# noveens/reviews4rec

Measured on AMD Instinct MI355X. Metric: train ratings/sec, higher is better.
Workload: dtype f32

## Files before the change

### include/r4r.h

```cpp
#ifndef R4R_H
#define R4R_H

#include <stddef.h>
#include <stdint.h>

#ifdef __cplusplus
extern "C" {
#endif

#define R4R_OK 0
#define R4R_ERR_ARG (-1)
#define R4R_ERR_LAUNCH (-2)
#define R4R_ERR_WORKSPACE (-3)

int r4r_version(void);
const char *r4r_last_error(void);

size_t r4r_textcnn_ws_bytes(int64_t N, int T, int E, int F, int64_t V);
int r4r_textcnn_fwd(const float *table, int64_t V, const int64_t *idx,
                    const float *conv_w, const float *conv_b,
                    float *pooled, int32_t *argmax,
                    void *ws, size_t ws_bytes,
                    int64_t N, int T, int E, int F, void *stream);

// ... 13 lines not shown
                      void *ws, size_t ws_bytes,
                      int64_t N, int T, int E, int F, void *stream);

int r4r_linear_fwd(const float *x, const float *w, const float *b, float *y,
                   int64_t N, int n_in, int n_out, int relu, void *stream);
size_t r4r_linear_bwd_ws_bytes(int64_t N, int n_in, int n_out);
int r4r_linear_bwd(const float *x, const float *w, const float *y, const float *g_y,
                   float *g_x, float *g_w, float *g_b, void *ws, size_t ws_bytes,
                   int64_t N, int n_in, int n_out, int relu, void *stream);

int r4r_dropout_fwd(const float *x, float *y, float *mult, int64_t n, float p,
                    uint64_t seed, uint64_t offset, uint64_t *offset_dev, void *stream);
int r4r_counter_add(uint64_t *counter, uint64_t delta, void *stream);
int r4r_mul(const float *a, const float *b, float *out, int64_t n, void *stream);
int r4r_add(const float *a, const float *b, float *out, int64_t n, void *stream);

int r4r_fm_fwd(const float *x, const float *V, const float *lin_w, const float *lin_b,
               float *out, int64_t N, int n, int k, void *stream);
int r4r_fm_bwd(const float *x, const float *V, const float *lin_w, const float *g_out,
               float *g_x, float *g_V, float *g_lin_w, float *g_lin_b,
               int64_t N, int n, int k, void *stream);

int r4r_embed_gather(const float *table, const int64_t *idx, float *out,
                     int64_t R, int D, int64_t n, void *stream);
int r4r_embed_scatter_add(const float *g_out, const int64_t *idx, float *g_table,
                          int64_t R, int D, int64_t n, void *stream);
int r4r_embed_scatter_add_ordered(const float *g_out, const int64_t *idx, float *g_table,
                                  int64_t R, int D, int64_t n, void *stream);

int r4r_rowdot_fwd(const float *a, const float *c, float *out, int64_t N, int D, void *stream);
int r4r_rowdot_bwd(const float *a, const float *c, const float *g_out, float *g_a, float *g_c,
                   int64_t N, int D, void *stream);
int r4r_bias_head_fwd(const float *r, const float *user_bias, const float *item_bias,
                      const float *global_bias, const int64_t *uid, const int64_t *iid,
                      float *out, int64_t N, void *stream);
int r4r_bias_head_bwd(const float *g_out, const int64_t *uid, const int64_t *iid,
                      float *g_user_bias, float *g_item_bias, float *g_global,
                      int64_t RU, int64_t RI, int64_t N, void *stream);

size_t r4r_narre_attn_ws_bytes(int64_t N, int R, int L);
int r4r_narre_attn_fwd(const float *x, const float *other, const float *W0, const float *b0,
                       const float *w3, const float *b3, const float *mult,
                       float *out, float *h_save, float *a_save,
                       int64_t N, int R, int L, void *stream);
int r4r_narre_attn_bwd(const float *x, const float *other, const float *W0, const float *w3,
                       const float *mult, const float *h_save, const float *a_save,
                       const float *g_out,
                       float *g_x, float *g_other, float *g_W0, float *g_b0, float *g_w3, float *g_b3,
                       void *ws, size_t ws_bytes,
                       int64_t N, int R, int L, void *stream);

int r4r_mse_fwd_bwd(const float *out, const float *y, float *se, float *g_out,
                    int64_t N, float denom, void *stream);

int r4r_sqdist_mean_fwd(const float *a, const float *b, float *out, int64_t N, int L, void *stream);
int r4r_sqdist_mean_bwd(const float *a, const float *b, const float *g_out, float *g_a, float *g_b,
                        int64_t N, int L, void *stream);

int r4r_adam_chunk_elems(void);
int r4r_adam_multi(int ntensor, const uint64_t *p, const uint64_t *g, const uint64_t *m, const uint64_t *v,
                   const int64_t *numel, float lr, double beta1, double beta2, float eps,
                   float weight_decay, int64_t step, const int64_t *step_dev, void *stream);
int r4r_adam_gathered(float *p, const float *gathered, int world, float *g_sum, float *m, float *v,
                      int64_t numel, float lr, double beta1, double beta2, float eps,
                      float weight_decay, int64_t step, void *stream);
int r4r_adam_gathered_guarded(float *p, const float *gathered, int world, float *g_sum, float *m, float *v,
                              int64_t numel, float lr, double beta1, double beta2, float eps,
                              float weight_decay, int64_t step, const uint32_t *abort_word, void *stream);

int r4r_peer_segment_create(int64_t bytes, void **ptr, uint8_t *handle);
int r4r_peer_segment_open(const uint8_t *handle, void **ptr);
int r4r_peer_segment_close(void *ptr);
int r4r_peer_segment_destroy(void *ptr);
int r4r_peer_push(const float *src, int64_t numel, const uint64_t *peer_dst, const uint64_t *peer_flags,
                  uint32_t *arrive, int rank, int world, uint32_t epoch, const uint32_t *wait_flags,
                  uint32_t *timed_out, double timeout_s, void *stream);
int r4r_peer_wait(const uint32_t *flags, int world, uint32_t epoch, uint32_t *timed_out, double timeout_s, void *stream);


#define R4R_CONV_AUTO 0
#define R4R_CONV_DIRECT 1
#define R4R_CONV_PROJECT 2
int r4r_deepconn_nparam(void);
int r4r_deepconn_layout(int E, int L, int64_t *offsets, int64_t *sizes, int64_t *total);
size_t r4r_deepconn_ws_bytes(int64_t B, int T, int E, int L, int64_t V);
size_t r4r_deepconn_ws_mult_offset(int64_t B, int T, int E, int L, int64_t V);
size_t r4r_deepconn_ws_count_offset(int64_t B, int T, int E, int L, int64_t V, int tower, int buffer);
int r4r_deepconn_step(const float *table, int64_t V, const int64_t *user_idx, const int64_t *item_idx,
                      const float *y, float *flat_p, float *flat_g,
                      float *pred, float *se, float *sse_accum,
                      void *ws, size_t ws_bytes,
                      int64_t B, int T, int E, int L,
                      float dropout_p, int training, uint64_t seed, uint64_t offset,
                      float inv_denom, int conv_algo, int token_buffer, int tokens_ready,
                      const int64_t *next_user_idx, const int64_t *next_item_idx,
                      float *flat_m, float *flat_v, float lr, double beta1, double beta2, float eps,
                      float weight_decay, int64_t adam_step, void *stream);
int r4r_deepconn_tokens(const int64_t *user_idx, const int64_t *item_idx, void *ws, size_t ws_bytes,
                        int64_t B, int T, int E, int L, int64_t V, int conv_algo, int token_buffer,
                        int discard, void *stream);

#define R4R_TIMING_TEXTCNN_FWD 0
#define R4R_TIMING_TEXTCNN_WGRAD 1
#define R4R_TIMING_ADAM 2
#define R4R_TIMING_PROJ_GEMM 3
#define R4R_TIMING_PROJ_GATHER 4
#define R4R_TIMING_SLOTS 8
int r4r_timing_enable(int slot_mask);
int r4r_timing_read(int slot, double *total_ms, int64_t *count, int reset);

size_t r4r_mf_ws_bytes(int64_t B, int D, int64_t n_users, int64_t n_items);
size_t r4r_mf_ws_persist_bytes(int64_t B, int D, int64_t n_users, int64_t n_items);
size_t r4r_mf_ws_mult_offset(int64_t B, int D, int64_t n_users, int64_t n_items);
size_t r4r_mf_ws_grad_offset(int64_t B, int D, int64_t n_users, int64_t n_items, int which);
int r4r_mf_step(const int64_t *uid, const int64_t *iid, const float *y,
                const uint64_t *p, const uint64_t *m, const uint64_t *v,
                int64_t n_users, int64_t n_items, int D,
                float *pred, float *se, float *sse_accum, void *ws, size_t ws_bytes, int64_t B,
                float dropout_p, int training, uint64_t seed, uint64_t offset, float inv_denom,
                int sweep_period, int64_t sweep_base, int sweep_all,
                float lr, double beta1, double beta2, float eps, float weight_decay, int64_t adam_step,
                void *stream);

int r4r_mf_rows_flush(const uint64_t *p, const uint64_t *m, const uint64_t *v,
                      int64_t n_users, int64_t n_items, int D, void *ws, size_t ws_bytes, int64_t B,
                      int sweep_period, int64_t sweep_base,
                      float lr, double beta1, double beta2, float eps, float weight_decay, int64_t adam_step,
                      void *stream);
size_t r4r_mf_ws_flag_offset(int64_t B, int D, int64_t n_users, int64_t n_items);

int r4r_sse_accumulate(const float *se, int64_t n, float *accum, void *stream);

size_t r4r_mf_dp_block_bytes(int64_t B_pad, int D);
int r4r_mf_grad(const int64_t *uid, const int64_t *iid, const float *y, const uint64_t *p,
                const uint64_t *m, const uint64_t *v,
                int64_t n_users, int64_t n_items, int D, float *pred, float *se, void *block, float *mult,
                int64_t B, int64_t B_pad, float dropout_p, int training, uint64_t seed, uint64_t offset,
                float inv_denom, void *ws, int sweep_period, int64_t sweep_base,
                float lr, double beta1, double beta2, float eps, float weight_decay, int64_t adam_step,
                void *stream);
int r4r_mf_apply(const void *blocks, int world, int64_t B_pad, const uint64_t *p, const uint64_t *m,
                 const uint64_t *v, int64_t n_users, int64_t n_items, int D, void *ws, size_t ws_bytes,
                 int sweep_period, int64_t sweep_base, int sweep_all,
                 const float *se, int64_t se_n, float *sse_accum,
                 float lr, double beta1, double beta2, float eps, float weight_decay, int64_t adam_step,
                 void *stream);
int r4r_mf_grad_push(const int64_t *uid, const int64_t *iid, const float *y, const uint64_t *p,
                     const uint64_t *m, const uint64_t *v,
                     int64_t n_users, int64_t n_items, int D, float *pred, float *se, float *mult,
                     int64_t B, int64_t B_pad, float dropout_p, int training, uint64_t seed, uint64_t offset,
                     float inv_denom, void *ws, int sweep_period, int64_t sweep_base,
                     float lr, double beta1, double beta2, float eps, float weight_decay, int64_t adam_step,
                     const uint64_t *peer_dst, const uint64_t *peer_flags, uint32_t *arrive, int rank, int world,
                     uint32_t epoch, void *stream);
int r4r_mf_apply_peer(const void *blocks, int world, int64_t B_pad, const uint64_t *p, const uint64_t *m,
                      const uint64_t *v, int64_t n_users, int64_t n_items, int D, void *ws, size_t ws_bytes,
                      int sweep_period, int64_t sweep_base, int sweep_all,
                      const float *se, int64_t se_n, float *sse_accum,
                      float lr, double beta1, double beta2, float eps, float weight_decay, int64_t adam_step,
                      const uint32_t *wait_flags, uint32_t epoch, uint32_t *timed_out, double timeout_s,
                      void *stream);

size_t r4r_dp_block_bytes(int nfields, const int *widths, int64_t B_pad);
int r4r_dp_pack(int nfields, const uint64_t *src, const int *widths, const int *pad_ones, int64_t n,
                int64_t B_pad, void *block, void *stream);
int r4r_dp_unpack(int nfields, const uint64_t *dst, const int *widths, const void *blocks, int world,
// ... 268 lines not shown
```

### reviews4rec_amd/csrc/engine.hip

```cpp
#include <stdlib.h>

#include "trace_device.h"
#include "textcnn.h"
#include "wgrad_device.h"
#include "tokens_device.h"
#include "adam_device.h"

namespace r4r {

constexpr int F_CONV = 100;
constexpr int FM_K = 8;
constexpr int MAX_L = 128;

enum { P_UCW = 0, P_UCB, P_UFW, P_UFB, P_ICW, P_ICB, P_IFW, P_IFB, P_FMV, P_FMLW, P_FMLB, P_GB, P_COUNT };

struct Layout {
    int64_t off[P_COUNT], size[P_COUNT], total;
};

static Layout make_layout(int E, int L) {
    Layout lay;
    const int64_t sz[P_COUNT] = {(int64_t)F_CONV * 3 * E, F_CONV, (int64_t)L * F_CONV, L,
                                 (int64_t)F_CONV * 3 * E, F_CONV, (int64_t)L * F_CONV, L,
                                 (int64_t)2 * L * FM_K, 2 * L, 1, 1};
    int64_t o = 0;
    for (int i = 0; i < P_COUNT; ++i) {
        lay.off[i] = o;
        lay.size[i] = sz[i];
        o += (sz[i] + 31) & ~(int64_t)31;
    }
    lay.total = o;
    return lay;
}

struct HeadArgs {
    const float *pmax[2]; const int *parg[2];
    const float *fc_w[2]; const float *fc_b[2];
    const float *V, *lin_w, *lin_b, *gbias;
    const float *y;
    float *pooled[2]; int *argmax[2];
    float *g_pooled[2];
    float *mult;
    float *x, *s, *g, *gz;
    float *pred, *se;
    int64_t B;
    int L, tiles, training, want_grad;
    float p_drop, inv_denom;
    uint64_t seed, offset;
};


constexpr int HEAD_MAX_TILES = 8;

#define SEL2(arr, s) ((s) ? (arr)[1] : (arr)[0])
HEAD_TRACE_DEFINE(r4r_debug_dc_head_trace)
template <int ML>
__global__ __launch_bounds__(256) void deepconn_head_wg_kernel(HeadArgs a) {
    HEAD_STAMP(0)
    constexpr int N2 = 2 * ML, PARTS = 256 / N2;
    __shared__ float sw[2][ML][F_CONV + 1];
    __shared__ float sfb[N2], slw[N2], sz[N2];
    __shared__ float sV[N2][FM_K];
    __shared__ float sp[2][F_CONV + 4];
    __shared__ float red[N2][PARTS + 1];
    const int tid = threadIdx.x, lane = tid & 63, w = tid >> 6;
    const int64_t b = blockIdx.x;
    const int L = a.L, n = 2 * L;
    const float lin_b0 = a.lin_b[0], gbias0 = a.gbias[0], yb = a.y ? a.y[b] : 0.f;

    constexpr int FQ = F_CONV / 4;
    typedef float hq4 __attribute__((ext_vector_type(4)));
    constexpr int WREGS = (2 * ML * FQ + 255) / 256;
    hq4 wreg[WREGS];
    const int wtot = 2 * L * FQ;
#pragma unroll
    for (int k = 0; k < WREGS; ++k) {
        const int i = min(tid + 256 * k, wtot - 1);
        const int t = i >= L * FQ;
        wreg[k] = *reinterpret_cast<const hq4 *>(SEL2(a.fc_w, t) + 4 * (i - t * L * FQ));
    }
    const int tn = min(tid, n - 1);
    const float fbreg = SEL2(a.fc_b, tn >= L)[tn - (tn >= L ? L : 0)];
    const float lwreg = a.lin_w[tn];
    constexpr int VREGS = (N2 * FM_K + 255) / 256;
    float vreg[VREGS];
#pragma unroll
    for (int k = 0; k < VREGS; ++k) vreg[k] = a.V[min(tid + 256 * k, n * FM_K - 1)];

    {
        const int t = w >> 1, f = lane + 64 * (w & 1), fc = min(f, F_CONV - 1);
        float best = -INFINITY;
        int bp = -1;
        if (a.tiles <= HEAD_MAX_TILES) {
            float v[HEAD_MAX_TILES];
            int pp[HEAD_MAX_TILES];
#pragma unroll
            for (int k = 0; k < HEAD_MAX_TILES; ++k) {
                const size_t o = ((size_t)b * a.tiles + min(k, a.tiles - 1)) * NP + fc;
                v[k] = SEL2(a.pmax, t)[o];
                pp[k] = SEL2(a.parg, t)[o];
            }
#pragma unroll
            for (int k = 0; k < HEAD_MAX_TILES; ++k)
                if (v[k] > best) { best = v[k]; bp = pp[k]; }
        } else {
            for (int k0 = 0; k0 < a.tiles; k0 += HEAD_MAX_TILES) {
                float v[HEAD_MAX_TILES];
                int pp[HEAD_MAX_TILES];
#pragma unroll
                for (int k = 0; k < HEAD_MAX_TILES; ++k) {
                    const bool in = k0 + k < a.tiles;
                    const size_t o = ((size_t)b * a.tiles + (in ? k0 + k : 0)) * NP + fc;
                    v[k] = in ? SEL2(a.pmax, t)[o] : -INFINITY;
                    pp[k] = SEL2(a.parg, t)[o];
                }
#pragma unroll
                for (int k = 0; k < HEAD_MAX_TILES; ++k)
                    if (v[k] > best) { best = v[k]; bp = pp[k]; }
            }
        }
        if (!(best > 0.f)) { best = 0.f; bp = -1; }
        if (f < F_CONV) {
            sp[t][f] = best;
            SEL2(a.pooled, t)[b * F_CONV + f] = best;
            SEL2(a.argmax, t)[b * F_CONV + f] = bp;
        }
    }
    HEAD_STAMP(1)
#pragma unroll
    for (int k = 0; k < WREGS; ++k) {
        const int i = tid + 256 * k;
        if (i < wtot) {
            const int t = i >= L * FQ, r = i - t * L * FQ, l = r / FQ, f0 = 4 * (r - l * FQ);
#pragma unroll
            for (int c = 0; c < 4; ++c) sw[t][l][f0 + c] = wreg[k][c];
        }
    }
    if (tid < n) { sfb[tid] = fbreg; slw[tid] = lwreg; }
#pragma unroll
    for (int k = 0; k < VREGS; ++k) {
// ... 19 lines not shown
        float xi[NI], mult[NI], lw[NI], gacc[NI];
#pragma unroll
        for (int u = 0; u < NI; ++u) {
            const int i = lane + 64 * u;
            xi[u] = 0.f; mult[u] = 1.f; gacc[u] = 0.f;
            lw[u] = (i < n) ? slw[i] : 0.f;
            if (i < n) {
                float acc = 0.f;
#pragma unroll
                for (int q = 0; q < PARTS; ++q) acc += red[i][q];
                xi[u] = acc + sfb[i];
            }
            if (a.training && a.p_drop > 0.f && i < n) {
                const uint32_t r = philox_first_word(a.offset + (uint64_t)(b * n + i), a.seed);
                const float uu = (float)(r >> 8) * (1.0f / 16777216.0f);
                mult[u] = (uu >= a.p_drop) ? 1.f / (1.f - a.p_drop) : 0.f;
            }
            xi[u] *= mult[u];
        }
        float inter = 0.f;
        float sk_keep[FM_K];
#pragma unroll
        for (int k = 0; k < FM_K; ++k) {
            float pv = 0.f, pv2 = 0.f, vv[NI];
#pragma unroll
            for (int u = 0; u < NI; ++u) {
                const int i = lane + 64 * u;
                vv[u] = (i < n) ? sV[i][k] : 0.f;
                pv += xi[u] * vv[u];
                pv2 += xi[u] * xi[u] * vv[u] * vv[u];
            }
            const float sk = wave_sum(pv);
            const float s2 = wave_sum(pv2);
            inter += sk * sk - s2;
#pragma unroll
            for (int u = 0; u < NI; ++u) gacc[u] += sk * vv[u] - xi[u] * vv[u] * vv[u];
            sk_keep[k] = sk;
        }
        float pl = 0.f;
#pragma unroll
        for (int u = 0; u < NI; ++u) pl += xi[u] * lw[u];
        const float lin = wave_sum(pl);
        const float pred = (0.5f * inter + lin + lin_b0) + gbias0;
        if (lane == 0) a.pred[b] = pred;
        if (has_y) {
            const float d = pred - yb;
            if (lane == 0) a.se[b] = d * d;
            if (want) {
                const float g = 2.f * d * a.inv_denom;
#pragma unroll
                for (int u = 0; u < NI; ++u) {
                    const int i = lane + 64 * u;
                    const float gx = g * (gacc[u] + lw[u]);
                    const float gz = gx * mult[u];
                    if (i < n) {
                        sz[i] = gz;
                        a.x[b * n + i] = xi[u];
                        a.gz[b * n + i] = gz;
                        a.mult[b * n + i] = mult[u];
                    }
                }
                if (lane < FM_K) {
                    float sv = 0.f;
#pragma unroll
                    for (int k = 0; k < FM_K; ++k) if (lane == k) sv = sk_keep[k];
                    a.s[b * FM_K + lane] = sv;
                }
                if (lane == 0) a.g[b] = g;
            }
        }
    }
    if (!want) return;
    __syncthreads();
    HEAD_STAMP(3)
    if (tid < 2 * F_CONV) {
        const int t = tid >= F_CONV, f = tid - t * F_CONV;
        float acc = 0.f;
        for (int l = 0; l < L; ++l) acc = fmaf(sz[t * L + l], sw[t][l][f], acc);
        SEL2(a.g_pooled, t)[b * F_CONV + f] = acc;
    }
    HEAD_STAMP(4)
}

struct HeadGradArgs {
    const float *pooled[2];
    const float *x, *s, *g, *gz;
    const float *V;
    const float *se;
    float *g_fc_w[2], *g_fc_b[2], *g_V, *g_lin_w, *g_lin_b, *g_gb;
    float *sse_accum;
    int64_t B;
    int L;
};

constexpr int HG_ROWS = 16, HG_COLS = 16;
__device__ __forceinline__ void head_grad_block(const HeadGradArgs &a, int blk) {
    __shared__ float red[HG_ROWS][HG_COLS];
    const int ox = threadIdx.x & (HG_COLS - 1), rg = threadIdx.x / HG_COLS;
    const int L = a.L, n = 2 * L;
    const int n_fcw = L * F_CONV;
    const int seg[9] = {n_fcw, L, n_fcw, L, n * FM_K, n, 1, 1, 1};
    int o = blk * HG_COLS + ox;
    int which = -1, local = 0, acc_o = o;
#pragma unroll
    for (int k = 0; k < 9; ++k) {
        if (which < 0) {
            if (acc_o < seg[k]) { which = k; local = acc_o; }
            else acc_o -= seg[k];
        }
    }
    float s = 0.f;
    if (which >= 0) {
        const bool is_w = which == 0 || which == 2, is_b = which == 1 || which == 3, is_v = which == 4, is_lw = which == 5;
        const int t = which >> 1;
        const int wl = local / F_CONV, wf = local - wl * F_CONV;
        const int vi = local / FM_K, vk = local - vi * FM_K;
        const float *pa = (is_w || is_b) ? a.gz : (which == 8 ? a.se : a.g);
        const int64_t sa = (is_w || is_b) ? n : 1;
        const int64_t oa = is_w ? t * L + wl : (is_b ? t * L + local : 0);
        const bool useb = is_w || is_v, usec = is_v || is_lw;
        const float *pb = is_w ? a.pooled[t & 1] : (is_v ? a.s : a.g);
        const int64_t sb = is_w ? F_CONV : (is_v ? FM_K : 1), ob = is_w ? wf : (is_v ? vk : 0);
        const float *pc = usec ? a.x : a.g;
        const int64_t sc = usec ? n : 1, oc = is_v ? vi : (is_lw ? local : 0);
        const float cv = is_v ? a.V[local] : 0.f;
        constexpr int HB = 8;
        for (int64_t b0 = rg; b0 < a.B; b0 += (int64_t)HG_ROWS * HB) {
            float va[HB], vb[HB], vc[HB];
#pragma unroll
            for (int k = 0; k < HB; ++k) {
                const int64_t b = min(b0 + (int64_t)k * HG_ROWS, a.B - 1);
                va[k] = pa[b * sa + oa];
                vb[k] = pb[b * sb + ob];
                vc[k] = pc[b * sc + oc];
            }
#pragma unroll
            for (int k = 0; k < HB; ++k) {
                const float B_ = useb ? vb[k] : 1.f, C_ = usec ? vc[k] : 1.f;
                const float term = va[k] * (B_ * C_ - C_ * C_ * cv);
                if (b0 + (int64_t)k * HG_ROWS < a.B) s += term;
            }
        }
    }
    red[rg][ox] = s;
    __syncthreads();
    if (rg == 0 && which >= 0) {
        float t = 0.f;
#pragma unroll
        for (int r = 0; r < HG_ROWS; ++r) t += red[r][ox];
        switch (which) {
            case 0: a.g_fc_w[0][local] = t; break;
            case 1: a.g_fc_b[0][local] = t; break;
            case 2: a.g_fc_w[1][local] = t; break;
            case 3: a.g_fc_b[1][local] = t; break;
            case 4: a.g_V[local] = t; break;
            case 5: a.g_lin_w[local] = t; break;
            case 6: a.g_lin_b[0] = t; break;
            case 7: a.g_gb[0] = t; break;
            default: if (a.sse_accum) a.sse_accum[0] += t; break;
        }
    }
}

BWD_TRACE_DEFINE(r4r_debug_dc_bwd_trace)
struct DcBackwardArgs {
    WgradArgs w;
    HeadGradArgs h;
    int hg_blocks;
    TokenArgs nx;
};
__global__ __launch_bounds__(WG_THREADS, 8) void deepconn_backward_kernel(DcBackwardArgs) {
    const DcBackwardArgs &A = kernel_args<DcBackwardArgs>();
    const WgradArgs &w = A.w;
    const HeadGradArgs &h = A.h;
    const TokenArgs &nx = A.nx;
    const int hg_blocks = A.hg_blocks;
    BWD_STAMP(0, wall_clock64())
    BWD_STAMP(2, (unsigned long long)blockIdx.z + 1)
    if (blockIdx.z == 1 || blockIdx.z == 2) {
        wgrad_block(w, blockIdx.x, blockIdx.y, blockIdx.z - 1);
    } else if (blockIdx.z == 0) {
        for (int blk = blockIdx.y * gridDim.x + blockIdx.x; blk < hg_blocks; blk += gridDim.x * gridDim.y) {
            head_grad_block(h, blk);
            __syncthreads();
        }
    } else {
        token_mark_block(nx, blockIdx.y * gridDim.x + blockIdx.x, gridDim.x * gridDim.y, WG_THREADS);
    }
#ifdef R4R_TRACE
    __syncthreads();
#endif
    BWD_STAMP(1, wall_clock64())
}

constexpr int RED_THREADS = 256;
struct FusedAdam {
    float *p, *m, *v;
    const float *g;
    int64_t lo[2], hi[2];
    AdamScalars s;
    int on;
};
__global__ __launch_bounds__(RED_THREADS) void deepconn_reduce_kernel(WgradArgs w, int red_blocks, int comp_blocks,
                                                                      TokenArgs nx, FusedAdam opt) {
    const int bx = blockIdx.x;
    if (bx < red_blocks) {
        const WgradTower &tw = w.t[blockIdx.y];
        const int nw = w.F * 3 * w.E;
        const int i = bx * RED_THREADS + threadIdx.x;
        const float *gp0 = i < nw ? tw.d_w + i : (i < nw + w.F ? tw.d_b + (i - nw) : nullptr);
        const int64_t o = gp0 ? gp0 - opt.g : 0;
        float P = 0.f, M = 0.f, V = 0.f;
        if (opt.on && gp0) { P = opt.p[o]; M = opt.m[o]; V = opt.v[o]; }
        float *dst;
        const float g = wgrad_reduce_elem(w, blockIdx.y, i, dst);
        if (opt.on && dst) {
            adam_elem(P, g, M, V, opt.s);
            opt.p[o] = P; opt.m[o] = M; opt.v[o] = V;
        }
    } else if (bx < red_blocks + comp_blocks) {
        token_compact_auto<RED_THREADS / 64>(nx.t[blockIdx.y], nx.V, bx - red_blocks);
    } else {
        const int64_t o = opt.lo[blockIdx.y] + (int64_t)(bx - red_blocks - comp_blocks) * RED_THREADS + threadIdx.x;
        if (o < opt.hi[blockIdx.y]) {
            float P = opt.p[o], M = opt.m[o], V = opt.v[o];
            adam_elem(P, opt.g[o], M, V, opt.s);
            opt.p[o] = P; opt.m[o] = M; opt.v[o] = V;
        }
    }
}

__global__ void sse_only_kernel(const float *__restrict__ se, float *__restrict__ accum, int64_t B) {
    __shared__ float red[256];
    float s = 0.f;
    for (int64_t i = threadIdx.x; i < B; i += 256) s += se[i];
    red[threadIdx.x] = s;
    __syncthreads();
    for (int off = 128; off > 0; off >>= 1) {
        if ((int)threadIdx.x < off) red[threadIdx.x] += red[threadIdx.x + off];
        __syncthreads();
    }
    if (threadIdx.x == 0) accum[0] += red[0];
}

struct StepWs {
    float *wp[2], *pmax[2]; int *parg[2];
    int *flags[2][2], *slot[2][2], *list[2][2], *count[2][2]; float *ptab[2];
    float *pooled[2]; int *argmax[2]; float *g_pooled[2];
    float *mult, *x, *s, *g, *gz;
    float *part_w[2], *part_b[2];
    size_t bytes;
};

static StepWs carve(void *ws, int64_t B, int T, int E, int L, int64_t V) {
    StepWs w;
    char *p = static_cast<char *>(ws);
    auto take = [&](size_t nbytes) { char *r = p; p += align256(nbytes); return r; };
    const size_t tiles128 = (size_t)(T + 2 + 127) / 128;
    const int ns = textcnn_wgrad_splits(B);
    for (int t = 0; t < 2; ++t) {
        w.wp[t] = reinterpret_cast<float *>(take(textcnn_wp_floats(E) * 4));
        w.pmax[t] = reinterpret_cast<float *>(take((size_t)B * tiles128 * NP * 4));
        w.parg[t] = reinterpret_cast<int *>(take((size_t)B * tiles128 * NP * 4));
        w.pooled[t] = reinterpret_cast<float *>(take((size_t)B * F_CONV * 4));
        w.argmax[t] = reinterpret_cast<int *>(take((size_t)B * F_CONV * 4));
        w.g_pooled[t] = reinterpret_cast<float *>(take((size_t)B * F_CONV * 4));
        w.part_w[t] = reinterpret_cast<float *>(take((size_t)ns * F_CONV * 3 * E * 4));
        w.part_b[t] = reinterpret_cast<float *>(take((size_t)ns * F_CONV * 4));
        for (int bf = 0; bf < 2; ++bf) {
            w.flags[bf][t] = reinterpret_cast<int *>(take((size_t)(V + 4) * 4));
            w.slot[bf][t] = reinterpret_cast<int *>(take((size_t)(V + 4) * 4));
            w.list[bf][t] = reinterpret_cast<int *>(take((size_t)proj_row_capacity(B, T, V) * 4));
            w.count[bf][t] = reinterpret_cast<int *>(take(256));
        }
        w.ptab[t] = reinterpret_cast<float *>(take(proj_ptab_floats(B, T, V) * 4));
    }
    w.mult = reinterpret_cast<float *>(take((size_t)B * 2 * L * 4));
    w.x = reinterpret_cast<float *>(take((size_t)B * 2 * L * 4));
    w.gz = reinterpret_cast<float *>(take((size_t)B * 2 * L * 4));
    w.s = reinterpret_cast<float *>(take((size_t)B * FM_K * 4));
    w.g = reinterpret_cast<float *>(take((size_t)B * 4));
    w.bytes = (size_t)(p - static_cast<char *>(ws));
    return w;
}

}

using namespace r4r;

extern "C" int r4r_deepconn_nparam(void) { return P_COUNT; }

extern "C" int r4r_deepconn_layout(int E, int L, int64_t *offsets, int64_t *sizes, int64_t *total) {
    R4R_REQUIRE(E > 0 && L > 0 && L <= MAX_L && offsets && sizes && total, "deepconn_layout: bad arguments");
    const Layout lay = make_layout(E, L);
    for (int i = 0; i < P_COUNT; ++i) { offsets[i] = lay.off[i]; sizes[i] = lay.size[i]; }
    *total = lay.total;
    return R4R_OK;
}

extern "C" size_t r4r_deepconn_ws_bytes(int64_t B, int T, int E, int L, int64_t V) {
    if (B < 0 || T <= 0 || E <= 0 || L <= 0 || V <= 0) return 0;
    return carve(nullptr, B, T, E, L, V).bytes;
}

extern "C" size_t r4r_deepconn_ws_mult_offset(int64_t B, int T, int E, int L, int64_t V) {
    char base[1];
    const StepWs w = carve(base, B, T, E, L, V);
    return (size_t)(reinterpret_cast<char *>(w.mult) - base);
}

extern "C" size_t r4r_deepconn_ws_count_offset(int64_t B, int T, int E, int L, int64_t V, int tower, int buffer) {
    char base[1];
    const StepWs w = carve(base, B, T, E, L, V);
    return (size_t)(reinterpret_cast<char *>(w.count[buffer & 1][tower & 1]) - base);
}

extern "C" int r4r_deepconn_tokens(const int64_t *user_idx, const int64_t *item_idx, void *ws, size_t ws_bytes,
                                   int64_t B, int T, int E, int L, int64_t V, int conv_algo, int token_buffer,
                                   int discard, void *stream) {
    R4R_REQUIRE(user_idx && item_idx && ws, "deepconn_tokens: null pointer");
    R4R_REQUIRE(token_buffer == 0 || token_buffer == 1, "deepconn_tokens: token_buffer must be 0 or 1");
    if (ws_bytes < r4r_deepconn_ws_bytes(B, T, E, L, V)) {
        set_error("deepconn_tokens: workspace %zu < %zu bytes", ws_bytes, r4r_deepconn_ws_bytes(B, T, E, L, V));
        return R4R_ERR_WORKSPACE;
    }
    if (B == 0 || textcnn_pick_algo(conv_algo, B, T, E, F_CONV) != R4R_CONV_PROJECT) return R4R_OK;
    const StepWs w = carve(ws, B, T, E, L, V);
    if (discard) {
        for (int t = 0; t < 2; ++t) (void)hipMemsetAsync(w.count[token_buffer][t], 0, sizeof(int), as_stream(stream));
        return check_launch("deepconn_tokens(discard)");
    }
    ProjTower pt[2];
    const int64_t *idx[2] = {user_idx, item_idx};
    for (int t = 0; t < 2; ++t) {
        pt[t] = ProjTower{};
        pt[t].idx = idx[t];
        pt[t].flags = w.flags[token_buffer][t]; pt[t].slot = w.slot[token_buffer][t];
        pt[t].list = w.list[token_buffer][t]; pt[t].count = w.count[token_buffer][t];
    }
    return textcnn_proj_tokens_launch(V, pt, 2, B, T, false, as_stream(stream));
}

extern "C" int r4r_deepconn_step(const float *table, int64_t V, const int64_t *user_idx, const int64_t *item_idx,
                                 const float *y, float *flat_p, float *flat_g,
                                 float *pred, float *se, float *sse_accum,
                                 void *ws, size_t ws_bytes,
                                 int64_t B, int T, int E, int L,
                                 float dropout_p, int training, uint64_t seed, uint64_t offset,
                                 float inv_denom, int conv_algo, int token_buffer, int tokens_ready,
                                 const int64_t *next_user_idx, const int64_t *next_item_idx,
                                 float *flat_m, float *flat_v, float lr, double beta1, double beta2, float eps,
                                 float weight_decay, int64_t adam_step,
                                 void *stream) {
    R4R_REQUIRE(table && user_idx && item_idx && flat_p && pred && ws, "deepconn_step: null pointer");
    R4R_REQUIRE(!flat_m == !flat_v, "deepconn_step: flat_m and flat_v go together");
    R4R_REQUIRE(!flat_m || (flat_g && adam_step >= 1), "deepconn_step: the fused optimiser needs gradients and "
                                                       "adam_step >= 1");
    R4R_REQUIRE(!next_user_idx == !next_item_idx, "deepconn_step: next_user_idx and next_item_idx go together");
    R4R_REQUIRE(!next_user_idx || flat_g, "deepconn_step: the next batch's tokens ride on the backward launches "
                                          "(training steps only)");
    R4R_REQUIRE(V > 0 && B >= 0 && T > 0, "deepconn_step: bad sizes");
    R4R_REQUIRE(E > 0 && E % 4 == 0, "deepconn_step: word_embed_size %d must be a positive multiple of 4", E);
    R4R_REQUIRE(L > 0 && L <= MAX_L, "deepconn_step: latent_size %d outside 1..%d", L, MAX_L);
    R4R_REQUIRE(!flat_g || (y && se), "deepconn_step: gradients need ratings y and the se buffer");
    R4R_REQUIRE(!y || se, "deepconn_step: se buffer required when y is given");
    R4R_REQUIRE(dropout_p >= 0.f && dropout_p < 1.f, "deepconn_step: dropout %f outside [0,1)", (double)dropout_p);
    R4R_REQUIRE(B * (int64_t)((T + 2 + 127) / 128) < (1ll << 31), "deepconn_step: grid too large");
    R4R_REQUIRE(token_buffer == 0 || token_buffer == 1, "deepconn_step: token_buffer must be 0 or 1");
    if (ws_bytes < r4r_deepconn_ws_bytes(B, T, E, L, V)) {
        set_error("deepconn_step: workspace %zu < %zu bytes", ws_bytes, r4r_deepconn_ws_bytes(B, T, E, L, V));
        return R4R_ERR_WORKSPACE;
    }
    if (B == 0) return R4R_OK;
    hipStream_t st = as_stream(stream);
    const Layout lay = make_layout(E, L);
    const StepWs w = carve(ws, B, T, E, L, V);
    const float *P[P_COUNT];
    float *G[P_COUNT];
    for (int i = 0; i < P_COUNT; ++i) {
        P[i] = flat_p + lay.off[i];
        G[i] = flat_g ? flat_g + lay.off[i] : nullptr;
    }

    const int64_t *idx[2] = {user_idx, item_idx};
    const int algo = textcnn_pick_algo(conv_algo, B, T, E, F_CONV);
    int tiles;
    if (algo == R4R_CONV_PROJECT) {
        ProjTower pt[2];
        for (int t = 0; t < 2; ++t) {
            pt[t].idx = idx[t];
            pt[t].conv_w = P[t ? P_ICW : P_UCW];
            pt[t].conv_b = P[t ? P_ICB : P_UCB];
            pt[t].flags = w.flags[token_buffer][t]; pt[t].slot = w.slot[token_buffer][t];
            pt[t].list = w.list[token_buffer][t]; pt[t].count = w.count[token_buffer][t];
            pt[t].ptab = w.ptab[t]; pt[t].pmax = w.pmax[t]; pt[t].parg = w.parg[t]; pt[t].wimg = w.wp[t];
        }
        if (!tokens_ready)
            if (int rc = textcnn_proj_tokens_launch(V, pt, 2, B, T, false, st)) return rc;
        if (int rc = textcnn_proj_compute_launch(table, V, pt, 2, B, T, E, F_CONV, st)) return rc;
        tiles = proj_tiles(T);
    } else {
        FwdTower ft[2];
        for (int t = 0; t < 2; ++t) {
            ft[t].idx = idx[t];
            ft[t].conv_w = P[t ? P_ICW : P_UCW];
            ft[t].conv_b = P[t ? P_ICB : P_UCB];
            ft[t].wp = w.wp[t]; ft[t].pmax = w.pmax[t]; ft[t].parg = w.parg[t];
        }
        if (int rc = textcnn_fwd_launch(table, ft, 2, B, T, E, F_CONV, st)) return rc;
        tiles = textcnn_tiles(T);
    }

    HeadArgs h;
    for (int t = 0; t < 2; ++t) {
        h.pmax[t] = w.pmax[t]; h.parg[t] = w.parg[t];
        h.fc_w[t] = P[t ? P_IFW : P_UFW]; h.fc_b[t] = P[t ? P_IFB : P_UFB];
        h.pooled[t] = w.pooled[t]; h.argmax[t] = w.argmax[t]; h.g_pooled[t] = w.g_pooled[t];
    }
    h.V = P[P_FMV]; h.lin_w = P[P_FMLW]; h.lin_b = P[P_FMLB]; h.gbias = P[P_GB];
    h.y = y; h.mult = w.mult; h.x = w.x; h.s = w.s; h.g = w.g; h.gz = w.gz;
    h.pred = pred; h.se = se;
    h.B = B; h.L = L; h.tiles = tiles; h.training = training; h.want_grad = flat_g != nullptr;
    h.p_drop = dropout_p; h.inv_denom = inv_denom; h.seed = seed; h.offset = offset;
    if (L <= 16) deepconn_head_wg_kernel<16><<<(unsigned)B, 256, 0, st>>>(h);
    else if (L <= 32) deepconn_head_wg_kernel<32><<<(unsigned)B, 256, 0, st>>>(h);
    else if (L <= 64) deepconn_head_wg_kernel<64><<<(unsigned)B, 256, 0, st>>>(h);
    else deepconn_head_wg_kernel<128><<<(unsigned)B, 256, 0, st>>>(h);

    if (!flat_g) {
        if (y && sse_accum) sse_only_kernel<<<1, 256, 0, st>>>(se, sse_accum, B);
        return check_launch("deepconn_step(forward)");
    }

    HeadGradArgs hg;
    for (int t = 0; t < 2; ++t) {
        hg.pooled[t] = w.pooled[t];
        hg.g_fc_w[t] = G[t ? P_IFW : P_UFW]; hg.g_fc_b[t] = G[t ? P_IFB : P_UFB];
    }
    hg.x = w.x; hg.s = w.s; hg.g = w.g; hg.gz = w.gz; hg.V = P[P_FMV]; hg.se = se;
    hg.g_V = G[P_FMV]; hg.g_lin_w = G[P_FMLW]; hg.g_lin_b = G[P_FMLB]; hg.g_gb = G[P_GB];
    hg.sse_accum = sse_accum; hg.B = B; hg.L = L;
    const int nout = 2 * (L * F_CONV + L) + 2 * L * FM_K + 2 * L + 3;
    const int hg_blocks = (nout + HG_COLS - 1) / HG_COLS;

    WgradTower wt[2];
    WgradArgs wa;
    for (int t = 0; t < 2; ++t) {
        wt[t].idx = idx[t]; wt[t].g_pooled = w.g_pooled[t]; wt[t].argmax = w.argmax[t];
        wt[t].part_w = w.part_w[t]; wt[t].part_b = w.part_b[t];
        wt[t].d_w = G[t ? P_ICW : P_UCW]; wt[t].d_b = G[t ? P_ICB : P_UCB];
    }
    for (int k = 0; k < MAX_TOWERS; ++k) wa.t[k] = wt[k < 2 ? k : 0];
    wa.table = table; wa.N = B; wa.T = T; wa.E = E; wa.F = F_CONV;
    wa.table_bytes = (int64_t)V * E * 4;
    wa.nsplit = textcnn_wgrad_splits(B);
    wa.per_split = (int)cdiv(B, wa.nsplit);
    const bool prefetch = next_user_idx && algo == R4R_CONV_PROJECT;
    TokenArgs nx{};
    if (prefetch) {
        ProjTower nt[2];
        const int64_t *nidx[2] = {next_user_idx, next_item_idx};
        const int ob = token_buffer ^ 1;
        for (int t = 0; t < 2; ++t) {
            nt[t] = ProjTower{};
            nt[t].idx = nidx[t];
            nt[t].flags = w.flags[ob][t]; nt[t].slot = w.slot[ob][t];
            nt[t].list = w.list[ob][t]; nt[t].count = w.count[ob][t];
        }
        nx = make_token_args(V, nt, 2, B, T);
    }
    {
        ScopedTiming tm(R4R_TIMING_TEXTCNN_WGRAD, st);
        deepconn_backward_kernel<<<dim3(F_CONV, wa.nsplit, prefetch ? 4 : 3), WG_THREADS, 0, st>>>(DcBackwardArgs{wa, hg, hg_blocks, nx});
    }
    const int red_blocks = (F_CONV * 3 * E + F_CONV + RED_THREADS - 1) / RED_THREADS;
    const int comp_blocks = prefetch ? (int)cdiv((V + 3) / 4, RED_THREADS * compact_groups(V)) : 0;
    FusedAdam opt{};
    int opt_blocks = 0;
    if (flat_m) {
        opt.on = 1;
        opt.p = flat_p; opt.m = flat_m; opt.v = flat_v; opt.g = flat_g;
        opt.lo[0] = lay.off[P_UFW]; opt.hi[0] = lay.off[P_ICW];
        opt.lo[1] = lay.off[P_IFW]; opt.hi[1] = lay.total;
        opt.s = adam_make_scalars(lr, beta1, beta2, eps, weight_decay, adam_step, nullptr);
        const int64_t longest = opt.hi[0] - opt.lo[0] > opt.hi[1] - opt.lo[1] ? opt.hi[0] - opt.lo[0] : opt.hi[1] - opt.lo[1];
        opt_blocks = (int)cdiv(longest, RED_THREADS);
    }
    deepconn_reduce_kernel<<<dim3(red_blocks + comp_blocks + opt_blocks, 2), RED_THREADS, 0, st>>>(
        wa, red_blocks, comp_blocks, nx, opt);
    return check_launch("deepconn_step");
}

extern "C" int r4r_sse_accumulate(const float *se, int64_t n, float *accum, void *stream) {
    R4R_REQUIRE(accum && (se || n == 0) && n >= 0, "sse_accumulate: bad arguments");
    if (n == 0) return R4R_OK;
    sse_only_kernel<<<1, 256, 0, as_stream(stream)>>>(se, accum, n);
    return check_launch("sse_accumulate");
}
```

### reviews4rec_amd/csrc/wgrad_device.h

```cpp
#pragma once
#include "textcnn.h"

namespace r4r {

typedef float wg_f32x4 __attribute__((ext_vector_type(4)));

constexpr int WG_THREADS = 256;

struct WgradArgs {
    WgradTower t[MAX_TOWERS];
    const float *table;
    int64_t N;
    int T, E, F, per_split, nsplit;
    int64_t table_bytes = 0;
};

constexpr int WG_CHUNK = 16;
constexpr int WG_FLIGHT = 8;

template <bool FIRST>
__device__ __forceinline__ void wgrad_block_pass(const WgradArgs &a, int f, int s, int tower, int v0,
                                                 long (&s_off)[WG_CHUNK][3], float (&s_g)[WG_CHUNK]) {
    const WgradTower &tw = a.t[tower];
    const float *__restrict__ table = a.table;
// ... 114 lines not shown
        if (live) {
            int pv[NRES];
            float gv[NRES];
#pragma unroll
            for (int k = 0; k < NRES; ++k) {
                const int i = lane + 64 * k, d = i / 3;
                const int64_t n = c0 + (d < nd ? d : 0);
                pv[k] = argmax[n * F + f];
                gv[k] = gp[n * F + f];
                if (d >= nd) pv[k] = -1;
            }
            long off[NRES], tokv[NRES];
            bool onv[NRES];
#pragma unroll
            for (int k = 0; k < NRES; ++k) {
                const int i = lane + 64 * k, d = i / 3, j = i - d * 3;
                const int64_t n = c0 + (d < nd ? d : 0);
                const int t = pv[k] - 2 + j;
                onv[k] = pv[k] >= 0 && t >= 0 && t < T;
                tokv[k] = idx[n * T + (onv[k] ? t : 0)];
            }
#pragma unroll
            for (int k = 0; k < NRES; ++k) asm volatile("" : "+v"(tokv[k]));
#pragma unroll
            for (int k = 0; k < NRES; ++k) off[k] = onv[k] ? tokv[k] * E : -1;
#pragma unroll
            for (int k = 0; k < NRES; ++k) {
                const int i = lane + 64 * k, d = i / 3, j = i - d * 3;
                if (d < WG_SUPER) {
                    p_off[wave][d][j] = off[k];
                    if (j == 0) p_g[wave][d] = pv[k] >= 0 ? gv[k] : 0.f;
                }
            }
        }
        __syncthreads();
        if (live && lane < nvec) {
            for (int r0 = 0; r0 < nd; r0 += WG_CHUNK) {
                wg_f32x4 v[WG_CHUNK];
#pragma unroll
                for (int d = 0; d < WG_CHUNK; ++d) {
                    const long off = p_off[wave][r0 + d][vj];
                    v[d] = *reinterpret_cast<const wg_f32x4 *>(table + (off < 0 ? 0 : off) + ve);
                }
#pragma unroll
                for (int d = 0; d < WG_CHUNK; ++d) {
                    const wg_f32x4 sum = acc + p_g[wave][r0 + d] * v[d];
                    acc = p_off[wave][r0 + d][vj] >= 0 ? sum : acc;
                }
            }
        }
        if (live && lane == 0)
            for (int d = 0; d < nd; ++d) sb += p_g[wave][d];
    }
    if (live && lane < nvec) *reinterpret_cast<wg_f32x4 *>(tw.part_w + ((size_t)s * F + f) * 3 * E + lane * 4) = acc;
    if (live && lane == 0) tw.part_b[(size_t)s * F + f] = sb;
}

constexpr int WG_MAX_SPLITS = 16;

__device__ __forceinline__ float wgrad_reduce_elem(const WgradArgs &a, int tower, int i, float *&dst) {
    const WgradTower &tw = a.t[tower];
    const int nw = a.F * 3 * a.E;
    const float *src;
    size_t stride;
    if (i < nw) { src = tw.part_w + i; stride = (size_t)nw; dst = tw.d_w + i; }
    else if (i < nw + a.F) { src = tw.part_b + (i - nw); stride = (size_t)a.F; dst = tw.d_b + (i - nw); }
    else { dst = nullptr; return 0.f; }
    float v[WG_MAX_SPLITS];
#pragma unroll
    for (int k = 0; k < WG_MAX_SPLITS; ++k) v[k] = src[(size_t)(k < a.nsplit ? k : 0) * stride];
    float s = 0.f;
#pragma unroll
    for (int k = 0; k < WG_MAX_SPLITS; ++k)
        if (k < a.nsplit) s += v[k];
    *dst = s;
    return s;
}

__device__ __forceinline__ void wgrad_reduce_block(const WgradArgs &a, int tower, int blk) {
    float *dst;
    (void)wgrad_reduce_elem(a, tower, blk * (int)blockDim.x + (int)threadIdx.x, dst);
}

}
```

Before: 1.391 million.

## Fuse DeepCoNN backward wgrad, split reduction, Adam and token compaction into one kernel

Adds a fused backward kernel that computes the conv weight gradient per filter and slice, reduces across splits in shared memory, and applies Adam in the same block. Head-gradient blocks also apply Adam inline, and token compaction runs in trailing blocks. Token marking for the next batch moves into extra blocks of the forward head kernel. The goal is to remove the separate reduce/Adam kernel launch and the global round trip of partial sums. The cost is that each block now loads the argmax offsets for all splits, and occupancy is bounded by a large block size. The fused path is on by default unless an env var or API call disables it.

```diff
diff --git a/include/r4r.h b/include/r4r.h
--- a/include/r4r.h
+++ b/include/r4r.h
@@ -119,6 +119,7 @@
 #define R4R_CONV_DIRECT 1
 #define R4R_CONV_PROJECT 2
 int r4r_deepconn_nparam(void);
+int r4r_deepconn_fused_wgrad(int requested);
 int r4r_deepconn_layout(int E, int L, int64_t *offsets, int64_t *sizes, int64_t *total);
 size_t r4r_deepconn_ws_bytes(int64_t B, int T, int E, int L, int64_t V);
 size_t r4r_deepconn_ws_mult_offset(int64_t B, int T, int E, int L, int64_t V);
diff --git a/reviews4rec_amd/csrc/engine.hip b/reviews4rec_amd/csrc/engine.hip
--- a/reviews4rec_amd/csrc/engine.hip
+++ b/reviews4rec_amd/csrc/engine.hip
@@ -47,6 +47,7 @@
     int L, tiles, training, want_grad;
     float p_drop, inv_denom;
     uint64_t seed, offset;
+    TokenArgs nx;
 };
 
 
@@ -56,6 +57,10 @@
 HEAD_TRACE_DEFINE(r4r_debug_dc_head_trace)
 template <int ML>
 __global__ __launch_bounds__(256) void deepconn_head_wg_kernel(HeadArgs a) {
+    if ((int64_t)blockIdx.x >= a.B) {
+        token_mark_block(a.nx, (int)(blockIdx.x - a.B), (int)(gridDim.x - a.B), 256);
+        return;
+    }
     HEAD_STAMP(0)
     constexpr int N2 = 2 * ML, PARTS = 256 / N2;
     __shared__ float sw[2][ML][F_CONV + 1];
@@ -241,6 +246,14 @@
     HEAD_STAMP(4)
 }
 
+struct FusedAdam {
+    float *p, *m, *v;
+    const float *g;
+    int64_t lo[2], hi[2];
+    AdamScalars s;
+    int on;
+};
+
 struct HeadGradArgs {
     const float *pooled[2];
     const float *x, *s, *g, *gz;
@@ -253,7 +266,8 @@
 };
 
 constexpr int HG_ROWS = 16, HG_COLS = 16;
-__device__ __forceinline__ void head_grad_block(const HeadGradArgs &a, int blk) {
+template <bool ADAM>
+__device__ __forceinline__ void head_grad_block(const HeadGradArgs &a, int blk, const FusedAdam *opt) {
     __shared__ float red[HG_ROWS][HG_COLS];
     const int ox = threadIdx.x & (HG_COLS - 1), rg = threadIdx.x / HG_COLS;
     const int L = a.L, n = 2 * L;
@@ -267,6 +281,15 @@
             if (acc_o < seg[k]) { which = k; local = acc_o; }
             else acc_o -= seg[k];
         }
+    }
+    int64_t po = -1;
+    float P = 0.f, M = 0.f, Vm = 0.f;
+    if (ADAM && rg == 0 && which >= 0 && which < 8) {
+        const float *gb = which == 0 ? a.g_fc_w[0] : which == 1 ? a.g_fc_b[0] : which == 2 ? a.g_fc_w[1]
+                        : which == 3 ? a.g_fc_b[1] : which == 4 ? a.g_V : which == 5 ? a.g_lin_w
+                        : which == 6 ? a.g_lin_b : a.g_gb;
+        po = (gb - opt->g) + local;
+        P = opt->p[po]; M = opt->m[po]; Vm = opt->v[po];
     }
     float s = 0.f;
     if (which >= 0) {
@@ -317,6 +340,10 @@
             case 6: a.g_lin_b[0] = t; break;
             case 7: a.g_gb[0] = t; break;
             default: if (a.sse_accum) a.sse_accum[0] += t; break;
+        }
+        if (ADAM && po >= 0) {
+            adam_elem(P, t, M, Vm, opt->s);
+            opt->p[po] = P; opt->m[po] = M; opt->v[po] = Vm;
         }
     }
 }
@@ -340,7 +367,7 @@
         wgrad_block(w, blockIdx.x, blockIdx.y, blockIdx.z - 1);
     } else if (blockIdx.z == 0) {
         for (int blk = blockIdx.y * gridDim.x + blockIdx.x; blk < hg_blocks; blk += gridDim.x * gridDim.y) {
-            head_grad_block(h, blk);
+            head_grad_block<false>(h, blk, nullptr);
             __syncthreads();
         }
     } else {
@@ -353,13 +380,6 @@
 }
 
 constexpr int RED_THREADS = 256;
-struct FusedAdam {
-    float *p, *m, *v;
-    const float *g;
-    int64_t lo[2], hi[2];
-    AdamScalars s;
-    int on;
-};
 __global__ __launch_bounds__(RED_THREADS) void deepconn_reduce_kernel(WgradArgs w, int red_blocks, int comp_blocks,
                                                                       TokenArgs nx, FusedAdam opt) {
     const int bx = blockIdx.x;
@@ -389,6 +409,46 @@
     }
 }
 
+struct DcFusedArgs {
+    WgradArgs w;
+    HeadGradArgs h;
+    TokenArgs nx;
+    FusedAdam opt;
+    int hg_blocks, nslice, sw, comp_blocks;
+};
+constexpr int FUSED_MAX_THREADS = WG_MAX_SPLITS * WGF_MAX_SW;
+#ifndef R4R_FUSED_WAVES
+#define R4R_FUSED_WAVES 5
+#endif
+__global__ __launch_bounds__(FUSED_MAX_THREADS, R4R_FUSED_WAVES) void deepconn_backward_fused_kernel(DcFusedArgs) {
+    const DcFusedArgs &A = kernel_args<DcFusedArgs>();
+    const int bx = blockIdx.x, hg_blocks = A.hg_blocks;
+    const int wg_blocks = 2 * A.w.F * A.nslice;
+    if (bx < hg_blocks) {
+        if (threadIdx.x >= HG_ROWS * HG_COLS) return;
+        if (A.opt.on) head_grad_block<true>(A.h, bx, &A.opt);
+        else head_grad_block<false>(A.h, bx, nullptr);
+    } else if (bx < hg_blocks + wg_blocks) {
+        const WgradArgs &w = A.w;
+        const FusedAdam &opt = A.opt;
+        const int i = bx - hg_blocks, nslice = A.nslice, sw = A.sw;
+        const int tower = i / (w.F * nslice), r = i - tower * w.F * nslice, f = r / nslice, slice = r - f * nslice;
+        float *dst = wgrad_fused_dst(w, tower, f, slice, sw);
+        const int64_t o = dst ? dst - opt.g : 0;
+        float P = 0.f, M = 0.f, V = 0.f;
+        if (opt.on && dst) { P = opt.p[o]; M = opt.m[o]; V = opt.v[o]; }
+        const float g = wgrad_fused_block(w, tower, f, slice, sw, dst);
+        if (opt.on && dst) {
+            adam_elem(P, g, M, V, opt.s);
+            opt.p[o] = P; opt.m[o] = M; opt.v[o] = V;
+        }
+    } else {
+        if (threadIdx.x >= RED_THREADS) return;
+        const int j = bx - hg_blocks - wg_blocks, tower = j / A.comp_blocks;
+        token_compact_auto<RED_THREADS / 64>(A.nx.t[tower], A.nx.V, j - tower * A.comp_blocks);
+    }
+}
+
 __global__ void sse_only_kernel(const float *__restrict__ se, float *__restrict__ accum, int64_t B) {
     __shared__ float red[256];
     float s = 0.f;
@@ -400,6 +460,16 @@
         __syncthreads();
     }
     if (threadIdx.x == 0) accum[0] += red[0];
+}
+
+static int g_dc_fused_request = -1;
+static bool dc_fused_wgrad() {
+    static int env = -1;
+    if (env < 0) {
+        const char *e = getenv("R4R_DC_FUSED_WGRAD");
+        env = (e && atoi(e) == 0) ? 0 : 1;
+    }
+    return g_dc_fused_request >= 0 ? g_dc_fused_request != 0 : env != 0;
 }
 
 struct StepWs {
@@ -448,6 +518,14 @@
 using namespace r4r;
 
 extern "C" int r4r_deepconn_nparam(void) { return P_COUNT; }
+
+extern "C" int r4r_deepconn_fused_wgrad(int requested) {
+    R4R_REQUIRE(requested >= -1 && requested <= 1, "deepconn_fused_wgrad: request %d (-1 environment, 0 off, 1 on)",
+                requested);
+    const int prev = g_dc_fused_request;
+    g_dc_fused_request = requested;
+    return prev;
+}
 
 extern "C" int r4r_deepconn_layout(int E, int L, int64_t *offsets, int64_t *sizes, int64_t *total) {
     R4R_REQUIRE(E > 0 && L > 0 && L <= MAX_L && offsets && sizes && total, "deepconn_layout: bad arguments");
@@ -570,38 +648,6 @@
         tiles = textcnn_tiles(T);
     }
 
-    HeadArgs h;
-    for (int t = 0; t < 2; ++t) {
-        h.pmax[t] = w.pmax[t]; h.parg[t] = w.parg[t];
-        h.fc_w[t] = P[t ? P_IFW : P_UFW]; h.fc_b[t] = P[t ? P_IFB : P_UFB];
-        h.pooled[t] = w.pooled[t]; h.argmax[t] = w.argmax[t]; h.g_pooled[t] = w.g_pooled[t];
-    }
-    h.V = P[P_FMV]; h.lin_w = P[P_FMLW]; h.lin_b = P[P_FMLB]; h.gbias = P[P_GB];
-    h.y = y; h.mult = w.mult; h.x = w.x; h.s = w.s; h.g = w.g; h.gz = w.gz;
-    h.pred = pred; h.se = se;
-    h.B = B; h.L = L; h.tiles = tiles; h.training = training; h.want_grad = flat_g != nullptr;
-    h.p_drop = dropout_p; h.inv_denom = inv_denom; h.seed = seed; h.offset = offset;
-    if (L <= 16) deepconn_head_wg_kernel<16><<<(unsigned)B, 256, 0, st>>>(h);
-    else if (L <= 32) deepconn_head_wg_kernel<32><<<(unsigned)B, 256, 0, st>>>(h);
-    else if (L <= 64) deepconn_head_wg_kernel<64><<<(unsigned)B, 256, 0, st>>>(h);
-    else deepconn_head_wg_kernel<128><<<(unsigned)B, 256, 0, st>>>(h);
-
-    if (!flat_g) {
-        if (y && sse_accum) sse_only_kernel<<<1, 256, 0, st>>>(se, sse_accum, B);
-        return check_launch("deepconn_step(forward)");
-    }
-
-    HeadGradArgs hg;
-    for (int t = 0; t < 2; ++t) {
-        hg.pooled[t] = w.pooled[t];
-        hg.g_fc_w[t] = G[t ? P_IFW : P_UFW]; hg.g_fc_b[t] = G[t ? P_IFB : P_UFB];
-    }
-    hg.x = w.x; hg.s = w.s; hg.g = w.g; hg.gz = w.gz; hg.V = P[P_FMV]; hg.se = se;
-    hg.g_V = G[P_FMV]; hg.g_lin_w = G[P_FMLW]; hg.g_lin_b = G[P_FMLB]; hg.g_gb = G[P_GB];
-    hg.sse_accum = sse_accum; hg.B = B; hg.L = L;
-    const int nout = 2 * (L * F_CONV + L) + 2 * L * FM_K + 2 * L + 3;
-    const int hg_blocks = (nout + HG_COLS - 1) / HG_COLS;
-
     WgradTower wt[2];
     WgradArgs wa;
     for (int t = 0; t < 2; ++t) {
@@ -628,20 +674,79 @@
         }
         nx = make_token_args(V, nt, 2, B, T);
     }
+    const int nvec = 3 * E / 4;
+    const bool fused = flat_g && dc_fused_wgrad() && nvec > 64 && nvec <= 2 * WG_THREADS && wa.table_bytes < (1ll << 32) &&
+                       wa.nsplit <= WG_MAX_SPLITS;
+    const int64_t mark_need = cdiv(B * (int64_t)T, 256);
+    const int mark_blocks = fused && prefetch ? (int)(mark_need < 256 ? mark_need : 256) : 0;
+
+    HeadArgs h;
+    for (int t = 0; t < 2; ++t) {
+        h.pmax[t] = w.pmax[t]; h.parg[t] = w.parg[t];
+        h.fc_w[t] = P[t ? P_IFW : P_UFW]; h.fc_b[t] = P[t ? P_IFB : P_UFB];
+        h.pooled[t] = w.pooled[t]; h.argmax[t] = w.argmax[t]; h.g_pooled[t] = w.g_pooled[t];
+    }
+    h.V = P[P_FMV]; h.lin_w = P[P_FMLW]; h.lin_b = P[P_FMLB]; h.gbias = P[P_GB];
+    h.y = y; h.mult = w.mult; h.x = w.x; h.s = w.s; h.g = w.g; h.gz = w.gz;
+    h.pred = pred; h.se = se;
+    h.B = B; h.L = L; h.tiles = tiles; h.training = training; h.want_grad = flat_g != nullptr;
+    h.p_drop = dropout_p; h.inv_denom = inv_denom; h.seed = seed; h.offset = offset;
+    h.nx = nx;
+    const unsigned head_grid = (unsigned)(B + mark_blocks);
+    if (L <= 16) deepconn_head_wg_kernel<16><<<head_grid, 256, 0, st>>>(h);
+    else if (L <= 32) deepconn_head_wg_kernel<32><<<head_grid, 256, 0, st>>>(h);
+    else if (L <= 64) deepconn_head_wg_kernel<64><<<head_grid, 256, 0, st>>>(h);
+    else deepconn_head_wg_kernel<128><<<head_grid, 256, 0, st>>>(h);
+
+    if (!flat_g) {
+        if (y && sse_accum) sse_only_kernel<<<1, 256, 0, st>>>(se, sse_accum, B);
+        return check_launch("deepconn_step(forward)");
+    }
+
+    HeadGradArgs hg;
+    for (int t = 0; t < 2; ++t) {
+        hg.pooled[t] = w.pooled[t];
+        hg.g_fc_w[t] = G[t ? P_IFW : P_UFW]; hg.g_fc_b[t] = G[t ? P_IFB : P_UFB];
+    }
+    hg.x = w.x; hg.s = w.s; hg.g = w.g; hg.gz = w.gz; hg.V = P[P_FMV]; hg.se = se;
+    hg.g_V = G[P_FMV]; hg.g_lin_w = G[P_FMLW]; hg.g_lin_b = G[P_FMLB]; hg.g_gb = G[P_GB];
+    hg.sse_accum = sse_accum; hg.B = B; hg.L = L;
+    const int nout = 2 * (L * F_CONV + L) + 2 * L * FM_K + 2 * L + 3;
+    const int hg_blocks = (nout + HG_COLS - 1) / HG_COLS;
+    FusedAdam opt{};
+    opt.g = flat_g;
+    if (flat_m) {
+        opt.on = 1;
+        opt.p = flat_p; opt.m = flat_m; opt.v = flat_v;
+        opt.lo[0] = lay.off[P_UFW]; opt.hi[0] = lay.off[P_ICW];
+        opt.lo[1] = lay.off[P_IFW]; opt.hi[1] = lay.total;
+        opt.s = adam_make_scalars(lr, beta1, beta2, eps, weight_decay, adam_step, nullptr);
+    }
+    const int comp_blocks = prefetch ? (int)cdiv((V + 3) / 4, RED_THREADS * compact_groups(V)) : 0;
+
+    if (fused) {
+        DcFusedArgs fa;
+        fa.w = wa; fa.h = hg; fa.nx = nx; fa.opt = opt;
+        fa.hg_blocks = hg_blocks;
+        fa.nslice = (int)cdiv(nvec, WGF_MAX_SW);
+        fa.sw = (int)cdiv(nvec, fa.nslice);
+        fa.comp_blocks = comp_blocks;
+        const int wg_threads = (wa.nsplit * fa.sw + 63) / 64 * 64;
+        const int threads = wg_threads > RED_THREADS ? wg_threads : RED_THREADS;
+        R4R_REQUIRE(threads <= FUSED_MAX_THREADS && threads >= 4 * fa.sw + 1, "deepconn_step: fused backward shape");
+        const int grid = hg_blocks + 2 * F_CONV * fa.nslice + 2 * comp_blocks;
+        ScopedTiming tm(R4R_TIMING_TEXTCNN_WGRAD, st);
+        deepconn_backward_fused_kernel<<<grid, threads, 0, st>>>(fa);
+        return check_launch("deepconn_step");
+    }
+
     {
         ScopedTiming tm(R4R_TIMING_TEXTCNN_WGRAD, st);
         deepconn_backward_kernel<<<dim3(F_CONV, wa.nsplit, prefetch ? 4 : 3), WG_THREADS, 0, st>>>(DcBackwardArgs{wa, hg, hg_blocks, nx});
     }
     const int red_blocks = (F_CONV * 3 * E + F_CONV + RED_THREADS - 1) / RED_THREADS;
-    const int comp_blocks = prefetch ? (int)cdiv((V + 3) / 4, RED_THREADS * compact_groups(V)) : 0;
-    FusedAdam opt{};
     int opt_blocks = 0;
     if (flat_m) {
-        opt.on = 1;
-        opt.p = flat_p; opt.m = flat_m; opt.v = flat_v; opt.g = flat_g;
-        opt.lo[0] = lay.off[P_UFW]; opt.hi[0] = lay.off[P_ICW];
-        opt.lo[1] = lay.off[P_IFW]; opt.hi[1] = lay.total;
-        opt.s = adam_make_scalars(lr, beta1, beta2, eps, weight_decay, adam_step, nullptr);
         const int64_t longest = opt.hi[0] - opt.lo[0] > opt.hi[1] - opt.lo[1] ? opt.hi[0] - opt.lo[0] : opt.hi[1] - opt.lo[1];
         opt_blocks = (int)cdiv(longest, RED_THREADS);
     }
diff --git a/reviews4rec_amd/csrc/wgrad_device.h b/reviews4rec_amd/csrc/wgrad_device.h
--- a/reviews4rec_amd/csrc/wgrad_device.h
+++ b/reviews4rec_amd/csrc/wgrad_device.h
@@ -220,4 +220,95 @@
     (void)wgrad_reduce_elem(a, tower, blk * (int)blockDim.x + (int)threadIdx.x, dst);
 }
 
-}
+#ifndef R4R_WGF_SW
+#define R4R_WGF_SW 48
+#endif
+constexpr int WGF_MAX_SW = R4R_WGF_SW;
+
+__device__ __forceinline__ float *wgrad_fused_dst(const WgradArgs &a, int tower, int f, int slice, int sw) {
+    const WgradTower &tw = a.t[tower];
+    const int tid = threadIdx.x, ncol = min(sw, 3 * a.E / 4 - slice * sw);
+    if (tid < 4 * ncol) return tw.d_w + (size_t)f * 3 * a.E + (size_t)slice * sw * 4 + tid;
+    if (slice == 0 && tid == 4 * ncol) return tw.d_b + f;
+    return nullptr;
+}
+
+__device__ __forceinline__ float wgrad_fused_block(const WgradArgs &a, int tower, int f, int slice, int sw, float *dst) {
+    __shared__ long f_off[WG_MAX_SPLITS][WG_CHUNK][3];
+    __shared__ float f_g[WG_MAX_SPLITS][WG_CHUNK];
+    __shared__ wg_f32x4 f_part[WG_MAX_SPLITS][WGF_MAX_SW];
+    __shared__ float f_pb[WG_MAX_SPLITS];
+    const WgradTower &tw = a.t[tower];
+    const int64_t *__restrict__ idx = tw.idx;
+    const float *__restrict__ gp = tw.g_pooled;
+    const int *__restrict__ argmax = tw.argmax;
+    const int T = a.T, E = a.E, F = a.F, nsplit = a.nsplit;
+    const int nvec = 3 * E / 4;
+    const int tid = threadIdx.x, nthr = blockDim.x;
+    const int s = tid / sw, c = tid - s * sw, v = slice * sw + c;
+    const bool live = s < nsplit && c < sw && v < nvec;
+    const int vj = (v * 4) / E, ve = v * 4 - vj * E;
+    const int64_t n0 = (int64_t)s * a.per_split;
+    const int64_t n1 = min(a.N, n0 + (int64_t)a.per_split);
+    const int rounds = (a.per_split + WG_CHUNK - 1) / WG_CHUNK;
+    const __amdgpu_buffer_rsrc_t rsrc =
+        __builtin_amdgcn_make_buffer_rsrc(const_cast<float *>(a.table), 0, (int)(unsigned)a.table_bytes, 0x00020000);
+    wg_f32x4 acc = (wg_f32x4){0.f, 0.f, 0.f, 0.f};
+    float sb = 0.f;
+    for (int r = 0; r < rounds; ++r) {
+        __syncthreads();
+        for (int i = tid; i < nsplit * WG_CHUNK * 3; i += nthr) {
+            const int rs = i / (WG_CHUNK * 3), d = (i - rs * WG_CHUNK * 3) / 3, j = i - rs * WG_CHUNK * 3 - d * 3;
+            const int64_t rn0 = (int64_t)rs * a.per_split + (int64_t)r * WG_CHUNK;
+            const int64_t rn1 = min(a.N, (int64_t)rs * a.per_split + (int64_t)a.per_split);
+            if (rn0 + d < rn1) {
+                const int64_t n = rn0 + d;
+                const int p = argmax[n * F + f];
+                const float gv = gp[n * F + f];
+                const int t = p - 2 + j;
+                long off = -1;
+                if (p >= 0 && t >= 0 && t < T) off = (long)idx[n * T + t] * E;
+                f_off[rs][d][j] = off;
+                if (j == 0) f_g[rs][d] = (p >= 0) ? gv : 0.f;
+            }
+        }
+        __syncthreads();
+        const int64_t c0 = n0 + (int64_t)r * WG_CHUNK;
+        const int nd = s < nsplit && c0 < n1 ? (int)min((int64_t)WG_CHUNK, n1 - c0) : 0;
+        if (live) {
+#pragma unroll
+            for (int d0 = 0; d0 < WG_CHUNK; d0 += WG_FLIGHT) {
+                wg_f32x4 row[WG_FLIGHT];
+                bool on[WG_FLIGHT];
+#pragma unroll
+                for (int u = 0; u < WG_FLIGHT; ++u) {
+                    const int d = d0 + u;
+                    const long off = d < nd ? f_off[s][d][vj] : -1;
+                    on[u] = off >= 0;
+                    const unsigned bo = on[u] ? (unsigned)((off + ve) * 4) : 0xfffffff0u;
+                    row[u] = __builtin_bit_cast(wg_f32x4, __builtin_amdgcn_raw_buffer_load_b128(rsrc, (int)bo, 0, 0));
+                }
+#pragma unroll
+                for (int u = 0; u < WG_FLIGHT; ++u) {
+                    const wg_f32x4 sum = acc + f_g[s][d0 + u < nd ? d0 + u : 0] * row[u];
+                    acc = on[u] ? sum : acc;
+                }
+            }
+        }
+        if (slice == 0 && c == 0 && s < nsplit)
+            for (int d = 0; d < nd; ++d) sb += f_g[s][d];
+    }
+    if (live) f_part[s][c] = acc;
+    if (slice == 0 && c == 0 && s < nsplit) f_pb[s] = sb;
+    __syncthreads();
+    if (!dst) return 0.f;
+    const bool is_w = tid < 4 * min(sw, nvec - slice * sw);
+    const float *src = is_w ? reinterpret_cast<const float *>(&f_part[0][0]) + tid : f_pb;
+    const int stride = is_w ? 4 * WGF_MAX_SW : 1;
+    float g = 0.f;
+    for (int k = 0; k < nsplit; ++k) g += src[k * stride];
+    *dst = g;
+    return g;
+}
+
+}
```

New measurement: 1.375 million (median of 2 runs). 0.988x the previous value.
